# PrimeIntellect-ai/prime

Measured on AMD Instinct MI355X. Metric: tokens_per_sec, higher is better.
Workload: dtype bf16; 1 GPU; model=intellect_10b, global_batch=8, seq_len=2048, parallelism=diloco1_h100_int8ring

## Files before the change

### prime_amd/models/llama.py

```python
from __future__ import annotations

import math

import torch
import torch.nn as nn
import torch.nn.functional as F
from torch.utils.checkpoint import checkpoint

from .. import ops
from .configs import LlamaConfig, get_config


class PrimeLinear(nn.Linear):

    def forward(self, x):
        return ops.tuned_linear(x, self.weight)


class RMSNorm(nn.Module):
    def __init__(self, dim: int, eps: float):
        super().__init__()
        self.weight = nn.Parameter(torch.ones(dim))
        self.eps = eps

    def forward(self, x):
        return ops.rmsnorm(x, self.weight, self.eps)


class Attention(nn.Module):
    def __init__(self, cfg: LlamaConfig):
        super().__init__()
        self.cfg = cfg
        hd = cfg.head_dim
        self.wqkv = PrimeLinear(cfg.dim, (cfg.n_heads + 2 * cfg.n_kv_heads) * hd, bias=False)
        self.wo = PrimeLinear(cfg.n_heads * hd, cfg.dim, bias=False)

    sp_group = None

    def forward(self, x, cos, sin, cache=None, pos: int = 0, pos_dev=None):
        B, S, _ = x.shape
        cfg = self.cfg
        hd = cfg.head_dim
        qkv = self.wqkv(x)
        q, k, v = qkv.split(
            [cfg.n_heads * hd, cfg.n_kv_heads * hd, cfg.n_kv_heads * hd], dim=-1
        )
        q = q.view(B, S, cfg.n_heads, hd)
        k = k.view(B, S, cfg.n_kv_heads, hd)
        v = v.view(B, S, cfg.n_kv_heads, hd)
        p32 = pos_dev["pos32"] if pos_dev is not None else None
        q = ops.apply_rope(q, cos, sin, pos_offset=pos, pos_dev=p32)
        k = ops.apply_rope(k, cos, sin, pos_offset=pos, pos_dev=p32)
        if cache is not None:
            kc, vc = cache
            if pos_dev is not None:
                kc.index_copy_(1, pos_dev["pos64"], k)
                vc.index_copy_(1, pos_dev["pos64"], v)
                o = ops.attn_decode(q, kc, vc, length=1,
                                    len_dev=pos_dev["len32"])
                return self.wo(o.reshape(B, 1, cfg.n_heads * hd))
            kc[:, pos : pos + S] = k
            vc[:, pos : pos + S] = v
            if S == 1:
                o = ops.attn_decode(q, kc, vc, length=pos + 1)
                return self.wo(o.reshape(B, 1, cfg.n_heads * hd))
            o = ops.flash_attention(q, k, v, causal=True)
            return self.wo(o.reshape(B, S, cfg.n_heads * hd))
        if self.sp_group is not None:
            from ..parallel.seqpar import ulysses_attention

            o = ulysses_attention(q, k, v, causal=True, group=self.sp_group)
        else:
            o = ops.flash_attention(q, k, v, causal=True)
        return self.wo(o.reshape(B, S, cfg.n_heads * hd))


class MLP(nn.Module):
    def __init__(self, cfg: LlamaConfig):
        super().__init__()
        self.w_gateup = PrimeLinear(cfg.dim, 2 * cfg.intermediate, bias=False)
        self.w_down = PrimeLinear(cfg.intermediate, cfg.dim, bias=False)

    def forward(self, x):
        return self.w_down(ops.swiglu(self.w_gateup(x)))


class Block(nn.Module):

    def __init__(self, cfg: LlamaConfig):
        super().__init__()
        self.attn_norm = RMSNorm(cfg.dim, cfg.norm_eps)
        self.attn = Attention(cfg)
        self.mlp_norm = RMSNorm(cfg.dim, cfg.norm_eps)
        self.mlp = MLP(cfg)

    def forward(self, x, res, cos, sin, cache=None, pos: int = 0, pos_dev=None):
        y, s = ops.fused_add_rmsnorm(x, res, self.attn_norm.weight,
                                     self.attn_norm.eps)
        a = self.attn(y, cos, sin, cache=cache, pos=pos, pos_dev=pos_dev)
        y2, s2 = ops.fused_add_rmsnorm(a, s, self.mlp_norm.weight,
                                       self.mlp_norm.eps)
        return self.mlp(y2), s2


class Llama(nn.Module):
    def __init__(self, cfg: LlamaConfig, activation_checkpointing: bool = False):
        super().__init__()
# ... 58 lines not shown
```

### prime_amd/ops/__init__.py

```python
from .functional import (
    apply_rope,
    invalidate_wt_cache,
    set_linear_fp8,
    set_linear_tuned,
    tuned_linear,
    attn_decode,
    fused_add_rmsnorm,
    cross_entropy,
    dequant_int8,
    flash_attention,
    fused_adamw,
    grad_sqnorm,
    mfma_probe,
    nesterov_outer,
    pseudograd,
    quant_int8,
    rmsnorm,
    swiglu,
    QBLK,
)
from . import reference
from ._lib import have_lib
from .build import build, LIB_PATH

__all__ = [
    "apply_rope",
    "attn_decode",
    "fused_add_rmsnorm",
# ... 18 lines not shown
```

### prime_amd/ops/_lib.py

```python
from __future__ import annotations

import ctypes
from typing import Optional

import torch

from .build import LIB_PATH, build, needs_build

_LIB: Optional[ctypes.CDLL] = None
_TRIED = False

_SIGS = {
    "prime_rmsnorm_fwd": [ctypes.c_void_p] * 5 + [ctypes.c_int64] * 2 + [ctypes.c_double],
    "prime_rmsnorm_bwd": [ctypes.c_void_p] * 7 + [ctypes.c_int64] * 3 + [ctypes.c_double],
    "prime_add_rmsnorm_fwd": [ctypes.c_void_p] * 7 + [ctypes.c_int64] * 2 + [ctypes.c_double],
    "prime_add_rmsnorm_bwd": [ctypes.c_void_p] * 8 + [ctypes.c_int64] * 3 + [ctypes.c_double],
    "prime_rope": [ctypes.c_void_p] * 5 + [ctypes.c_int64] * 4 + [ctypes.c_int, ctypes.c_int64, ctypes.c_void_p],
    "prime_swiglu_fwd": [ctypes.c_void_p] * 3 + [ctypes.c_int64] * 2,
    "prime_swiglu_bwd": [ctypes.c_void_p] * 4 + [ctypes.c_int64] * 2,
    "prime_adamw": [ctypes.c_void_p] * 7 + [ctypes.c_int64] + [ctypes.c_double] * 5 + [ctypes.c_int64],
    "prime_grad_sqnorm": [ctypes.c_void_p] * 3 + [ctypes.c_int64] * 2,
    "prime_grad_sqnorm_partials": [],
    "prime_pseudograd": [ctypes.c_void_p] * 4 + [ctypes.c_int64],
    "prime_quant_int8": [ctypes.c_void_p] * 4 + [ctypes.c_int64],
    "prime_dequant_int8": [ctypes.c_void_p] * 4 + [ctypes.c_int64] * 2,
    "prime_nesterov_outer": [ctypes.c_void_p] * 6 + [ctypes.c_int64] + [ctypes.c_double] * 2,
    "prime_cross_entropy": [ctypes.c_void_p] * 5 + [ctypes.c_int64] * 2 + [ctypes.c_double] + [ctypes.c_int64] * 2,
    "prime_flash_fwd": [ctypes.c_void_p] * 6 + [ctypes.c_int64] * 5 + [ctypes.c_double] + [ctypes.c_int64] * 7,
    "prime_attn_delta": [ctypes.c_void_p] * 4 + [ctypes.c_int64] * 2,
    "prime_flash_bwd_dq": [ctypes.c_void_p] * 9 + [ctypes.c_int64] * 5 + [ctypes.c_double] + [ctypes.c_int64] * 10,
    "prime_flash_bwd_dkv": [ctypes.c_void_p] * 13 + [ctypes.c_int64] * 6 + [ctypes.c_double] + [ctypes.c_int64] * 10,
    "prime_mfma_probe": [ctypes.c_void_p] * 4,
    "prime_mfma_probe32": [ctypes.c_void_p] * 4,
    "prime_transpose_bshd": [ctypes.c_void_p] * 3 + [ctypes.c_int64] * 7,
    "prime_attn_decode": [ctypes.c_void_p] * 5 + [ctypes.c_int64] * 6 + [ctypes.c_double, ctypes.c_void_p],
    "prime_gemm_nt": [ctypes.c_void_p] * 4 + [ctypes.c_int64] * 4,
    "prime_gemm_nt8": [ctypes.c_void_p] * 4 + [ctypes.c_int64] * 4,
    "prime_quant_fp8": [ctypes.c_void_p] * 6 + [ctypes.c_int64] * 2,
    "prime_rowwise_quant_fp8": [ctypes.c_void_p] * 4 + [ctypes.c_int64] * 3,
    "prime_transpose_fp8": [ctypes.c_void_p] * 3 + [ctypes.c_int64] * 7 + [ctypes.c_void_p] * 3 + [ctypes.c_int64],
# ... 60 lines not shown
```

### prime_amd/ops/csrc/cross_entropy.hip

```cpp
#include "common.h"

__global__ void ce_fwd_bwd_kernel(const bf16* __restrict__ logits,
                                  const int32_t* __restrict__ targets,
                                  float* __restrict__ loss,
                                  bf16* __restrict__ dlogits, int64_t R, int V,
                                  float grad_scale, int ignore_index,
                                  int compute_grad) {
  __shared__ float red_m[256];
  __shared__ float red_s[256];
  const int tid = threadIdx.x;
  const int nthr = blockDim.x;
  const int vv = V / 8;
  for (int64_t r = blockIdx.x; r < R; r += gridDim.x) {
    const int tgt = targets[r];
    if (tgt == ignore_index) {
      if (tid == 0) loss[r] = 0.f;
      if (compute_grad) {
        bf16x8 z{};
#pragma unroll
        for (int j = 0; j < 8; ++j) z.v[j] = f2bf(0.f);
        bf16x8* dr = reinterpret_cast<bf16x8*>(dlogits + r * V);
        for (int i = tid; i < vv; i += nthr) dr[i] = z;
      }
      continue;
    }
    const bf16x8* zr = reinterpret_cast<const bf16x8*>(logits + r * V);
    float m = -INFINITY, s = 0.f;
    for (int i = tid; i < vv; i += nthr) {
      const bf16x8 z = zr[i];
#pragma unroll
      for (int j = 0; j < 8; ++j) {
        const float f = bf2f(z.v[j]);
        if (f > m) {
          s = s * __expf(m - f) + 1.f;
          m = f;
        } else {
          s += __expf(f - m);
        }
      }
    }
    red_m[tid] = m;
    red_s[tid] = s;
    __syncthreads();
    for (int stride = nthr / 2; stride > 0; stride >>= 1) {
      if (tid < stride) {
        const float m2 = red_m[tid + stride], s2 = red_s[tid + stride];
        const float mm = fmaxf(red_m[tid], m2);
        red_s[tid] = red_s[tid] * __expf(red_m[tid] - mm) + s2 * __expf(m2 - mm);
        red_m[tid] = mm;
      }
      __syncthreads();
    }
    const float M = red_m[0], S = red_s[0];
    __syncthreads();
    if (tid == 0) loss[r] = M + __logf(S) - bf2f(logits[r * V + tgt]);
    if (compute_grad) {
      const float invS = 1.f / S;
      bf16x8* dr = reinterpret_cast<bf16x8*>(dlogits + r * V);
      for (int i = tid; i < vv; i += nthr) {
        const bf16x8 z = zr[i];
        bf16x8 d;
#pragma unroll
        for (int j = 0; j < 8; ++j) {
          const int col = i * 8 + j;
          float p = __expf(bf2f(z.v[j]) - M) * invS;
          if (col == tgt) p -= 1.f;
          d.v[j] = f2bf(p * grad_scale);
        }
        dr[i] = d;
      }
    }
  }
// ... 16 lines not shown
```

### prime_amd/ops/csrc/rope.hip

```cpp
#include "common.h"

__global__ void rope_kernel(const bf16* __restrict__ x, bf16* __restrict__ y,
                            const float* __restrict__ cos_t,
                            const float* __restrict__ sin_t, int64_t nrows,
                            int H, int S, int D, float sign,
                            int64_t pos_offset,
                            const int* __restrict__ pos_dev) {
  if (pos_dev) pos_offset = *pos_dev;
  const int half = D / 2;
  const int hv = half / 4;
  const int64_t total = nrows * hv;
  for (int64_t idx = (int64_t)blockIdx.x * blockDim.x + threadIdx.x;
       idx < total; idx += (int64_t)gridDim.x * blockDim.x) {
    const int64_t row = idx / hv;
    const int i4 = (int)(idx - row * hv) * 4;
    const int64_t s = (row / H) % S + pos_offset;
    const bf16x4 x1 = *reinterpret_cast<const bf16x4*>(x + row * D + i4);
    const bf16x4 x2 = *reinterpret_cast<const bf16x4*>(x + row * D + half + i4);
    const f32x4v c = *reinterpret_cast<const f32x4v*>(cos_t + s * half + i4);
    const f32x4v sn = *reinterpret_cast<const f32x4v*>(sin_t + s * half + i4);
    bf16x4 y1, y2;
#pragma unroll
    for (int j = 0; j < 4; ++j) {
      const float a = bf2f(x1.v[j]), b = bf2f(x2.v[j]);
      const float sj = sign * sn.v[j];
      y1.v[j] = f2bf(a * c.v[j] - b * sj);
      y2.v[j] = f2bf(b * c.v[j] + a * sj);
    }
    *reinterpret_cast<bf16x4*>(y + row * D + i4) = y1;
    *reinterpret_cast<bf16x4*>(y + row * D + half + i4) = y2;
  }
}

PRIME_API int prime_rope(hipStream_t stream, const void* x, void* y,
                         const void* cos_t, const void* sin_t, int64_t nrows,
                         int64_t H, int64_t S, int64_t D, int backward,
                         int64_t pos_offset, const void* pos_dev) {
  if (D % 8 != 0) return hipErrorInvalidValue;
  int64_t total = nrows * (D / 8);
  int grid = prime_grid(total, 256);
  hipLaunchKernelGGL(rope_kernel, dim3(grid), dim3(256), 0, stream,
                     (const bf16*)x, (bf16*)y, (const float*)cos_t,
                     (const float*)sin_t, nrows, (int)H, (int)S, (int)D,
                     backward ? -1.f : 1.f, pos_offset, (const int*)pos_dev);
  return (int)hipGetLastError();
}
```

### prime_amd/ops/csrc/swiglu.hip

```cpp
#include "common.h"

__device__ __forceinline__ float sigmoidf_(float x) {
  return 1.f / (1.f + __expf(-x));
}

__global__ void swiglu_fwd_kernel(const bf16* __restrict__ gu,
                                  bf16* __restrict__ out, int64_t R, int I) {
  const int iv = I / 8;
  const int64_t total = R * iv;
  for (int64_t idx = (int64_t)blockIdx.x * blockDim.x + threadIdx.x;
       idx < total; idx += (int64_t)gridDim.x * blockDim.x) {
    const int64_t r = idx / iv;
    const int i = (int)(idx - r * iv) * 8;
    const bf16x8 g = *reinterpret_cast<const bf16x8*>(gu + r * 2 * I + i);
    const bf16x8 u = *reinterpret_cast<const bf16x8*>(gu + r * 2 * I + I + i);
    bf16x8 o;
#pragma unroll
    for (int j = 0; j < 8; ++j) {
      const float gf = bf2f(g.v[j]);
      o.v[j] = f2bf(gf * sigmoidf_(gf) * bf2f(u.v[j]));
    }
    *reinterpret_cast<bf16x8*>(out + r * I + i) = o;
  }
}

__global__ void swiglu_bwd_kernel(const bf16* __restrict__ dout,
                                  const bf16* __restrict__ gu,
                                  bf16* __restrict__ dgu, int64_t R, int I) {
  const int iv = I / 8;
  const int64_t total = R * iv;
  for (int64_t idx = (int64_t)blockIdx.x * blockDim.x + threadIdx.x;
       idx < total; idx += (int64_t)gridDim.x * blockDim.x) {
    const int64_t r = idx / iv;
    const int i = (int)(idx - r * iv) * 8;
    const bf16x8 g = *reinterpret_cast<const bf16x8*>(gu + r * 2 * I + i);
    const bf16x8 u = *reinterpret_cast<const bf16x8*>(gu + r * 2 * I + I + i);
    const bf16x8 d = *reinterpret_cast<const bf16x8*>(dout + r * I + i);
    bf16x8 dg, du;
#pragma unroll
    for (int j = 0; j < 8; ++j) {
      const float gf = bf2f(g.v[j]);
      const float sg = sigmoidf_(gf);
      const float silu = gf * sg;
      const float df = bf2f(d.v[j]);
      dg.v[j] = f2bf(df * bf2f(u.v[j]) * sg * (1.f + gf * (1.f - sg)));
      du.v[j] = f2bf(df * silu);
    }
    *reinterpret_cast<bf16x8*>(dgu + r * 2 * I + i) = dg;
    *reinterpret_cast<bf16x8*>(dgu + r * 2 * I + I + i) = du;
  }
}

PRIME_API int prime_swiglu_fwd(hipStream_t stream, const void* gu, void* out,
                               int64_t R, int64_t I) {
  if (I % 8 != 0) return hipErrorInvalidValue;
  int grid = prime_grid(R * (I / 8), 256);
  hipLaunchKernelGGL(swiglu_fwd_kernel, dim3(grid), dim3(256), 0, stream,
                     (const bf16*)gu, (bf16*)out, R, (int)I);
  return (int)hipGetLastError();
}

PRIME_API int prime_swiglu_bwd(hipStream_t stream, const void* dout,
                               const void* gu, void* dgu, int64_t R, int64_t I) {
  if (I % 8 != 0) return hipErrorInvalidValue;
  int grid = prime_grid(R * (I / 8), 256);
  hipLaunchKernelGGL(swiglu_bwd_kernel, dim3(grid), dim3(256), 0, stream,
                     (const bf16*)dout, (const bf16*)gu, (bf16*)dgu, R, (int)I);
  return (int)hipGetLastError();
}
```

### prime_amd/ops/functional.py

```python
from __future__ import annotations

import torch

from . import reference as ref
from ._lib import check, lib, ptr, stream_of

_DW_ROWS = 1024


def _is_hip(t: torch.Tensor) -> bool:
    return t.is_cuda


class _RMSNorm(torch.autograd.Function):
    @staticmethod
    def forward(ctx, x: torch.Tensor, w: torch.Tensor, eps: float):
        if not _is_hip(x):
            ctx.save_for_backward(x, w)
            ctx.eps = eps
            return ref.rmsnorm(x, w, eps)
        x = x.contiguous()
        shp = x.shape
        D = shp[-1]
        if D % 8 != 0:
# ... 30 lines not shown
        dx = torch.empty_like(x)
        G = max(1, min(R, _DW_ROWS))
        dw = torch.empty(G, D, device=x.device, dtype=torch.float32)
        check(
            lib().prime_rmsnorm_bwd(
                stream_of(x), ptr(dy), ptr(x), ptr(w), ptr(rstd), ptr(dx), ptr(dw), R, D, G, ctx.eps
            ),
            "rmsnorm_bwd",
        )
        return dx, dw.sum(0).to(w.dtype), None


def rmsnorm(x: torch.Tensor, w: torch.Tensor, eps: float = 1e-5) -> torch.Tensor:
    return _RMSNorm.apply(x, w, eps)


class _Rope(torch.autograd.Function):
    @staticmethod
    def forward(ctx, x, cos, sin, pos_offset: int, pos_dev=None):
        if not _is_hip(x):
            ctx.cpu = (cos, sin, pos_offset)
            return ref.apply_rope(x, cos, sin, pos_offset)
        ctx.cpu = None
        x = x.contiguous()
        B, S, H, D = x.shape
        y = torch.empty_like(x)
        check(
            lib().prime_rope(
                stream_of(x), ptr(x), ptr(y), ptr(cos), ptr(sin), B * S * H,
                H, S, D, 0, pos_offset, ptr(pos_dev),
            ),
            "rope_fwd",
        )
        ctx.save_for_backward(cos, sin)
        ctx.meta = (B, S, H, D, pos_offset)
        return y

    @staticmethod
    def backward(ctx, dy):
        if ctx.cpu is not None:
            cos, sin, off = ctx.cpu
            return ref.apply_rope(dy, cos, -sin, off), None, None, None, None
        cos, sin = ctx.saved_tensors
        B, S, H, D, off = ctx.meta
        dy = dy.contiguous()
        dx = torch.empty_like(dy)
        check(
            lib().prime_rope(
                stream_of(dy), ptr(dy), ptr(dx), ptr(cos), ptr(sin), B * S * H,
                H, S, D, 1, off, ptr(None),
            ),
            "rope_bwd",
        )
        return dx, None, None, None, None


def apply_rope(x, cos, sin, pos_offset: int = 0, pos_dev=None):
    return _Rope.apply(x, cos, sin, pos_offset, pos_dev)


class _SwiGLU(torch.autograd.Function):
    @staticmethod
    def forward(ctx, gu):
        if not _is_hip(gu):
            ctx.save_for_backward(gu)
            return ref.swiglu(gu)
        gu = gu.contiguous()
        I = gu.shape[-1] // 2
        if I % 8 != 0:
            raise NotImplementedError(
                f"swiglu kernel needs intermediate dim % 8 == 0 (got {I})"
            )
        R = gu.numel() // (2 * I)
        out = torch.empty(*gu.shape[:-1], I, device=gu.device, dtype=gu.dtype)
        check(lib().prime_swiglu_fwd(stream_of(gu), ptr(gu), ptr(out), R, I), "swiglu_fwd")
        ctx.save_for_backward(gu)
        return out

    @staticmethod
    def backward(ctx, dout):
        (gu,) = ctx.saved_tensors
        if not _is_hip(gu):
            g = gu.detach().float().requires_grad_(True)
            with torch.enable_grad():
                y = ref.swiglu(g)
            (gx,) = torch.autograd.grad(y, [g], dout.float())
            return gx.to(gu.dtype)
        dout = dout.contiguous()
        I = gu.shape[-1] // 2
        R = gu.numel() // (2 * I)
        dgu = torch.empty_like(gu)
        check(lib().prime_swiglu_bwd(stream_of(gu), ptr(dout), ptr(gu), ptr(dgu), R, I), "swiglu_bwd")
        return dgu


def swiglu(gu: torch.Tensor) -> torch.Tensor:
    return _SwiGLU.apply(gu)


def transpose_bshd(x: torch.Tensor) -> torch.Tensor:
    B, S, H, D = x.shape
    if not x.is_cuda or S % 64 != 0 or D % 64 != 0 or x.stride(3) != 1:
        return x.permute(0, 2, 3, 1).contiguous()
    out = torch.empty(B, H, D, S, device=x.device, dtype=x.dtype)
    check(
        lib().prime_transpose_bshd(
            stream_of(x), ptr(x), ptr(out), B, S, H, D,
            x.stride(0), x.stride(1), x.stride(2),
        ),
        "transpose_bshd",
    )
    return out


def _bshd_ok(t: torch.Tensor) -> bool:
    sb, ss, sh, sd = t.stride()
    return sd == 1 and sb % 8 == 0 and ss % 8 == 0 and sh % 8 == 0 \
        and t.storage_offset() % 8 == 0


def _check_flash_shape(S: int, D: int) -> None:
    if D not in (64, 128) or S % 64 != 0:
# ... 160 lines not shown
    M, C = x2.shape
    st = _FP8_ACT.get(site)
    import os

    fused_ok = os.environ.get("PRIME_AMD_FUSED_TQ", "0") == "1"
    if st is None or M % 64 or C % 128 or not fused_ok:
        xt = transpose_bshd(x2.view(1, M, C // 128, 128)).view(C, M)
        return _quant_act_fp8(xt, site, e5m2=e5m2)
    dt8 = torch.float8_e5m2 if e5m2 else torch.float8_e4m3fn
    xt8 = torch.empty(C, M, device=x2.device, dtype=dt8)
    st["next"].zero_()
    check(
        lib().prime_transpose_fp8(
            stream_of(x2), ptr(x2), ptr(xt8), 1, M, C // 128, 128,
            x2.stride(0) * M, x2.stride(0), 128,
            ptr(st["amax"]), ptr(st["next"]), ptr(st["sinv"]), 1 if e5m2 else 0,
        ),
        "transpose_fp8",
    )
    st["amax"], st["next"] = st["next"], st["amax"]
    return xt8, st["sinv"]


def _compute_dw(x2, w, dy2):
    N, K = w.shape
    M = x2.shape[0]
    if N % 128 == 0 and M % 64 == 0 and M >= 4096:
        if (_LINEAR_FP8_WGRAD and K % 128 == 0 and M % 16 == 0
                and x2.dtype == torch.bfloat16):
            xt8, xtinv = _transpose_quant_fp8(
                x2, ("xT", w.data_ptr(), *w.shape))
            dyt8, dytinv = _transpose_quant_fp8(
                dy2, ("dyT", w.data_ptr(), *w.shape), e5m2=True)
            g = torch._scaled_mm(xt8, dyt8.t(), scale_a=xtinv,
                                 scale_b=dytinv, out_dtype=x2.dtype)
            return transpose_bshd(g.view(1, K, N // 128, 128)).view(N, K)
        dyt = transpose_bshd(dy2.view(1, M, N // 128, 128)).view(N, M)
        return torch.mm(dyt, x2)
    return torch.mm(dy2.t(), x2)


def _linear_backward(x2, w, dy):
    N, K = w.shape
    M = x2.shape[0]
    dy2 = dy.reshape(-1, N).contiguous()
    wt = _wt_of(w) if _LINEAR_TUNED else None
    if (_LINEAR_FP8_DGRAD and wt is not None and M % 16 == 0
            and dy2.dtype == torch.bfloat16):
        dy8, dyinv = _quant_act_fp8(dy2, ("dy", w.data_ptr(), *w.shape),
                                    e5m2=True)
        wt8, wtinv = _w8_of(wt, skey=("wt", w.data_ptr(), *w.shape))
        dx = torch._scaled_mm(dy8, wt8.t(), scale_a=dyinv, scale_b=wtinv,
                              out_dtype=dy2.dtype)
    elif wt is not None:
        dx = torch.matmul(dy2, wt.t())
    else:
        dx = torch.matmul(dy2, w)
    return dx.view(*dy.shape[:-1], K), _compute_dw(x2, w, dy2)


class _TunedLinear(torch.autograd.Function):
    @staticmethod
# ... 98 lines not shown
class _Fp8Linear(torch.autograd.Function):
    @staticmethod
    def forward(ctx, x, w):
        x2 = x.reshape(-1, x.shape[-1]).contiguous()
        rw = _fp8_rowwise_on()
        if rw:
            x8, sxinv = _quant_rowwise_fp8(x2)
        else:
            x8, sxinv = _quant_act_fp8(x2, (w.data_ptr(), *w.shape))
        w8, swinv = _w8_of(w, rowwise=rw)
        y = torch._scaled_mm(x8, w8.t(), scale_a=sxinv, scale_b=swinv,
                             out_dtype=x.dtype)
        ctx.save_for_backward(x2, w)
        return y.view(*x.shape[:-1], w.shape[0])

    @staticmethod
    def backward(ctx, dy):
        x2, w = ctx.saved_tensors
        return _linear_backward(x2, w, dy)


def tuned_linear(x: torch.Tensor, w: torch.Tensor) -> torch.Tensor:
    if not _is_hip(x) or x.numel() // x.shape[-1] < 1024:
        return torch.nn.functional.linear(x, w)
    if _LINEAR_FP8 and x.shape[-1] % 16 == 0 and w.shape[0] % 16 == 0:
        return _Fp8Linear.apply(x, w)
    return _TunedLinear.apply(x, w)


def fused_adamw(p32, p16, grad, m, v, *, lr, beta1, beta2, eps, wd, step,
                gscale=None):
    check(
        lib().prime_adamw(
            stream_of(p32), ptr(p32), ptr(p16), ptr(grad), ptr(m), ptr(v),
            ptr(gscale), p32.numel(), lr, beta1, beta2, eps, wd, step,
        ),
        "adamw",
    )


def grad_sqnorm(grad: torch.Tensor, out: torch.Tensor) -> None:
    part = torch.zeros(lib().prime_grad_sqnorm_partials(), device=grad.device,
                       dtype=torch.float32)
    check(lib().prime_grad_sqnorm(stream_of(grad), ptr(grad), ptr(part),
                                  grad.numel(), part.numel()),
          "grad_sqnorm")
    out.add_(part.sum())


def pseudograd(outer32, master32, out_delta):
# ... 139 lines not shown
```

### prime_amd/parallel/flat.py

```python
from __future__ import annotations

from typing import Iterator

import torch
import torch.nn as nn

from .. import ops

ALIGN = 64


class FlatParamSpace:

    def __init__(self, module: nn.Module):
        self.module = module
        self.params: list[tuple[str, nn.Parameter]] = [
            (n, p) for n, p in module.named_parameters() if p.requires_grad
        ]
        if not self.params:
            raise ValueError("module has no trainable parameters")
        seen: dict[int, str] = {}
        uniq = []
        for n, p in self.params:
            if id(p) in seen:
# ... 3 lines not shown
        self.params = uniq

        dev = self.params[0][1].device
        dt = self.params[0][1].dtype
        self.device, self.dtype = dev, dt

        self.offsets: dict[str, tuple[int, int, torch.Size]] = {}
        off = 0
        for n, p in self.params:
            numel = p.numel()
            self.offsets[n] = (off, numel, p.shape)
            off += (numel + ALIGN - 1) // ALIGN * ALIGN
        self.numel_padded = off

        self.flat_w = torch.zeros(off, device=dev, dtype=dt)
        self.flat_grad = torch.zeros(off, device=dev, dtype=dt)
        for n, p in self.params:
            o, k, shp = self.offsets[n]
            self.flat_w[o : o + k].copy_(p.detach().flatten())
            p.data = self.flat_w[o : o + k].view(shp)
            p.grad = self.flat_grad[o : o + k].view(shp)
        self.master32 = self.flat_w.float()
        self._sq = None

    def zero_grad(self) -> None:
        self.flat_grad.zero_()

    def grad_views(self) -> Iterator[torch.Tensor]:
        for n, _ in self.params:
            o, k, shp = self.offsets[n]
            yield self.flat_grad[o : o + k].view(shp)

    def clip_grad_norm_(self, max_norm: float) -> torch.Tensor:
        norm = self.flat_grad.float().norm(2)
        scale = (max_norm / (norm + 1e-6)).clamp(max=1.0)
        self.flat_grad.mul_(scale.to(self.flat_grad.dtype))
        return norm

    def grad_clip_scale(self, max_norm: float) -> torch.Tensor:
        if self._sq is None:
            self._sq = torch.zeros(1, device=self.device, dtype=torch.float32)
        self._sq.zero_()
        ops.grad_sqnorm(self.flat_grad, self._sq)
        return (max_norm / (self._sq.sqrt() + 1e-6)).clamp(max=1.0)

    def state_dict(self) -> dict:
        return {"flat_w": self.flat_w, "master32": self.master32}

    def load_flat_(self, master32: torch.Tensor) -> None:
        self.master32.copy_(master32)
        self.flat_w.copy_(self.master32.to(self.dtype))
        ops.invalidate_wt_cache()


class FusedAdamW:

    def __init__(self, flat: FlatParamSpace, lr=3e-4, betas=(0.9, 0.95),
                 eps=1e-8, weight_decay=0.1):
        self.flat = flat
        self.lr, self.betas, self.eps, self.wd = lr, betas, eps, weight_decay
        self.m = torch.zeros_like(flat.master32)
        self.v = torch.zeros_like(flat.master32)
        self.step_count = 0

    def step(self, gscale=None) -> None:
# ... 30 lines not shown
```

### prime_amd/train.py

```python
from __future__ import annotations

import math
import os
import time
from pathlib import Path

import torch

from .ckpt.manager import CheckpointManager
from .data import DataConfig, build_dataloader
from .models import build_model
from .parallel.diloco import DilocoOptimizer
from .parallel.flat import FlatParamSpace, FusedAdamW
from .parallel.mesh import ElasticDeviceMesh, MeshConfig
from .utils.config import TrainConfig
from .utils.logging import JsonLogger
from .utils.metrics import MetricsWriter, model_flops_per_token, mfu


def lr_at(step: int, cfg) -> float:
    if step < cfg.warmup_steps:
        return cfg.lr * (step + 1) / max(1, cfg.warmup_steps)
    if not cfg.lr_decay_steps:
        return cfg.lr
# ... 67 lines not shown
        if self.fsdp:
            from .parallel.fsdp import ShardedParamSpace

            if not cfg.model.activation_checkpointing:
                self.model.activation_checkpointing = True
            self.flat = ShardedParamSpace(self.model, self.mesh)
            if self.mesh.outer_group is not None:
                import torch.distributed as dist

                dist.broadcast(self.flat.flat_w, src=self.mesh.worker_rank,
                               group=self.mesh.outer_group)
                self.flat.master32.copy_(self.flat.flat_w.float())
        else:
            self.flat = FlatParamSpace(self.model)
            if self.mesh.initialized:
                import torch.distributed as dist

                dist.broadcast(self.flat.flat_w, src=0)
                self.flat.master32.copy_(self.flat.flat_w.float())

        from . import ops as _ops

        _ops.set_linear_tuned(self.device.type == "cuda" and not self.fsdp)
        _ops.set_linear_fp8(cfg.model.fp8 and self.device.type == "cuda",
                            dgrad=cfg.model.fp8_dgrad,
                            wgrad=cfg.model.fp8_wgrad)

        self.inner = FusedAdamW(
            self.flat, lr=cfg.optim.lr, betas=tuple(cfg.optim.betas),
            eps=cfg.optim.eps, weight_decay=cfg.optim.weight_decay,
        )
        self.elastic = None
        self.shard_client = None
        if cfg.parallel.elastic and self.mesh.is_leader:
            from .parallel.elastic import ElasticWorker

            self.elastic = ElasticWorker(
                worker_name=cfg.run_name,
                host_store=os.environ.get("PRIME_GLOBAL_HOST", "0") == "1",
                heartbeat_interval=cfg.parallel.heartbeat_interval,
                heartbeat_timeout=cfg.parallel.heartbeat_timeout,
                ckpt_provider=lambda: self.diloco.live_state(),
            )
        elif cfg.parallel.elastic and self.fsdp:
            from .parallel.elastic import ElasticShardClient

# ... 60 lines not shown
            cfg.data.micro_batch_size * cfg.data.grad_accum * cfg.model.seq_len
            * max(1, self.mesh.world_size)
        )
        self.flops_per_token = model_flops_per_token(self.model_cfg, cfg.model.seq_len)

    def train_step(self) -> torch.Tensor:
        cfg = self.cfg
        self.inner.lr = lr_at(self.step_count, cfg.optim)
        self.flat.zero_grad()
        loss_acc = None
        for _ in range(cfg.data.grad_accum):
            x, y = self.data.next_batch(self.device)
            if self.seq_par:
                sl = cfg.model.seq_len
                r = self.mesh.worker_rank
                x = x[:, r * sl : (r + 1) * sl]
                y = y[:, r * sl : (r + 1) * sl]
            loss = self.model.loss(x, y) / cfg.data.grad_accum
            loss.backward()
            loss_acc = loss.detach() if loss_acc is None else loss_acc + loss.detach()
        if self.fsdp:
            self.flat.finalize_grads()
        else:
            self.mesh.local_allreduce_grad(self.flat.flat_grad)
        gscale = None
        if cfg.optim.grad_clip > 0:
            if self.device.type == "cuda" and not self.fsdp:
                gscale = self.flat.grad_clip_scale(cfg.optim.grad_clip)
            else:
                self.flat.clip_grad_norm_(cfg.optim.grad_clip)
        did_outer = self.diloco.step(gscale)
        self.step_count += 1
        if did_outer:
            self._maybe_checkpoint()
        return loss_acc

    def _maybe_checkpoint(self) -> None:
        if not self.ckpt or self.cfg.checkpoint.interval <= 0:
            return
        if self.diloco.outer_step_count % self.cfg.checkpoint.interval != 0:
            return
        if not (self.mesh.is_leader or self.fsdp):
            return
        self.save_checkpoint()

    def save_checkpoint(self) -> None:
# ... 175 lines not shown
```

Baseline: 16120 tokens/s.

## Fuse QKV rope and gate-up SwiGLU backward with transposed grads; write wgrads directly

Adds fused autograd paths for the QKV projection plus RoPE and the gate-up projection plus SwiGLU. Their backward kernels produce the packed gradient and its transpose in one pass, so the weight-gradient GEMM can consume it without a separate transpose. Linear weight gradients are written directly into slots of the flat gradient buffer, which skips a full zero of that buffer and an extra accumulate copy. The cost is more complex gradient bookkeeping (zero ranges, deferred finalize), with a risk of stale or wrong gradients if a slot is not cleared correctly.

```diff
diff --git a/prime_amd/models/llama.py b/prime_amd/models/llama.py
--- a/prime_amd/models/llama.py
+++ b/prime_amd/models/llama.py
@@ -41,6 +41,17 @@
         B, S, _ = x.shape
         cfg = self.cfg
         hd = cfg.head_dim
+        if cache is None and pos_dev is None:
+            q, k, v = ops.qkv_rope(x, self.wqkv.weight, cos, sin,
+                                   cfg.n_heads, cfg.n_kv_heads, hd,
+                                   pos_offset=pos)
+            if self.sp_group is not None:
+                from ..parallel.seqpar import ulysses_attention
+
+                o = ulysses_attention(q, k, v, causal=True, group=self.sp_group)
+            else:
+                o = ops.flash_attention(q, k, v, causal=True)
+            return self.wo(o.reshape(B, S, cfg.n_heads * hd))
         qkv = self.wqkv(x)
         q, k, v = qkv.split(
             [cfg.n_heads * hd, cfg.n_kv_heads * hd, cfg.n_kv_heads * hd], dim=-1
@@ -82,7 +93,7 @@
         self.w_down = PrimeLinear(cfg.intermediate, cfg.dim, bias=False)
 
     def forward(self, x):
-        return self.w_down(ops.swiglu(self.w_gateup(x)))
+        return self.w_down(ops.gateup_swiglu(x, self.w_gateup.weight))
 
 
 class Block(nn.Module):
diff --git a/prime_amd/ops/__init__.py b/prime_amd/ops/__init__.py
--- a/prime_amd/ops/__init__.py
+++ b/prime_amd/ops/__init__.py
@@ -3,7 +3,14 @@
     invalidate_wt_cache,
     set_linear_fp8,
     set_linear_tuned,
+    set_direct_wgrad,
+    direct_wgrad_enabled,
     tuned_linear,
+    gateup_swiglu,
+    qkv_rope,
+    qkv_grad_pack,
+    rope_packed_fwd,
+    swiglu_bwd_t,
     attn_decode,
     fused_add_rmsnorm,
     cross_entropy,
diff --git a/prime_amd/ops/_lib.py b/prime_amd/ops/_lib.py
--- a/prime_amd/ops/_lib.py
+++ b/prime_amd/ops/_lib.py
@@ -16,6 +16,9 @@
     "prime_add_rmsnorm_fwd": [ctypes.c_void_p] * 7 + [ctypes.c_int64] * 2 + [ctypes.c_double],
     "prime_add_rmsnorm_bwd": [ctypes.c_void_p] * 8 + [ctypes.c_int64] * 3 + [ctypes.c_double],
     "prime_rope": [ctypes.c_void_p] * 5 + [ctypes.c_int64] * 4 + [ctypes.c_int, ctypes.c_int64, ctypes.c_void_p],
+    "prime_rope_strided": [ctypes.c_void_p] * 5 + [ctypes.c_int64] * 7,
+    "prime_qkv_grad_pack": [ctypes.c_void_p] * 8 + [ctypes.c_int64] * 6,
+    "prime_swiglu_bwd_t": [ctypes.c_void_p] * 5 + [ctypes.c_int64] * 2,
     "prime_swiglu_fwd": [ctypes.c_void_p] * 3 + [ctypes.c_int64] * 2,
     "prime_swiglu_bwd": [ctypes.c_void_p] * 4 + [ctypes.c_int64] * 2,
     "prime_adamw": [ctypes.c_void_p] * 7 + [ctypes.c_int64] + [ctypes.c_double] * 5 + [ctypes.c_int64],
diff --git a/prime_amd/ops/csrc/cross_entropy.hip b/prime_amd/ops/csrc/cross_entropy.hip
--- a/prime_amd/ops/csrc/cross_entropy.hip
+++ b/prime_amd/ops/csrc/cross_entropy.hip
@@ -46,8 +46,10 @@
       if (tid < stride) {
         const float m2 = red_m[tid + stride], s2 = red_s[tid + stride];
         const float mm = fmaxf(red_m[tid], m2);
-        red_s[tid] = red_s[tid] * __expf(red_m[tid] - mm) + s2 * __expf(m2 - mm);
-        red_m[tid] = mm;
+        if (mm > -INFINITY) {
+          red_s[tid] = red_s[tid] * __expf(red_m[tid] - mm) + s2 * __expf(m2 - mm);
+          red_m[tid] = mm;
+        }
       }
       __syncthreads();
     }
diff --git a/prime_amd/ops/csrc/rope.hip b/prime_amd/ops/csrc/rope.hip
--- a/prime_amd/ops/csrc/rope.hip
+++ b/prime_amd/ops/csrc/rope.hip
@@ -1,4 +1,12 @@
 #include "common.h"
+
+__device__ __forceinline__ void rope_rot(bf16 x1, bf16 x2, float c, float sn,
+                                         float sign, bf16& y1, bf16& y2) {
+  const float a = bf2f(x1), b = bf2f(x2);
+  const float sj = sign * sn;
+  y1 = f2bf(a * c - b * sj);
+  y2 = f2bf(b * c + a * sj);
+}
 
 __global__ void rope_kernel(const bf16* __restrict__ x, bf16* __restrict__ y,
                             const float* __restrict__ cos_t,
@@ -21,12 +29,8 @@
     const f32x4v sn = *reinterpret_cast<const f32x4v*>(sin_t + s * half + i4);
     bf16x4 y1, y2;
 #pragma unroll
-    for (int j = 0; j < 4; ++j) {
-      const float a = bf2f(x1.v[j]), b = bf2f(x2.v[j]);
-      const float sj = sign * sn.v[j];
-      y1.v[j] = f2bf(a * c.v[j] - b * sj);
-      y2.v[j] = f2bf(b * c.v[j] + a * sj);
-    }
+    for (int j = 0; j < 4; ++j)
+      rope_rot(x1.v[j], x2.v[j], c.v[j], sn.v[j], sign, y1.v[j], y2.v[j]);
     *reinterpret_cast<bf16x4*>(y + row * D + i4) = y1;
     *reinterpret_cast<bf16x4*>(y + row * D + half + i4) = y2;
   }
@@ -45,3 +49,141 @@
                      backward ? -1.f : 1.f, pos_offset, (const int*)pos_dev);
   return (int)hipGetLastError();
 }
+
+__global__ void rope_strided_kernel(const bf16* __restrict__ x,
+                                    bf16* __restrict__ y,
+                                    const float* __restrict__ cos_t,
+                                    const float* __restrict__ sin_t,
+                                    int64_t nrows, int H, int S, int D,
+                                    int64_t in_stride, int64_t head_off,
+                                    float sign, int64_t pos_offset) {
+  const int half = D / 2;
+  const int hv = half / 4;
+  const int64_t total = nrows * hv;
+  for (int64_t idx = (int64_t)blockIdx.x * blockDim.x + threadIdx.x;
+       idx < total; idx += (int64_t)gridDim.x * blockDim.x) {
+    const int64_t row = idx / hv;
+    const int i4 = (int)(idx - row * hv) * 4;
+    const int64_t tok = row / H;
+    const int h = (int)(row - tok * H);
+    const int64_t s = tok % S + pos_offset;
+    const bf16* xr = x + tok * in_stride + head_off + (int64_t)h * D;
+    const bf16x4 x1 = *reinterpret_cast<const bf16x4*>(xr + i4);
+    const bf16x4 x2 = *reinterpret_cast<const bf16x4*>(xr + half + i4);
+    const f32x4v c = *reinterpret_cast<const f32x4v*>(cos_t + s * half + i4);
+    const f32x4v sn = *reinterpret_cast<const f32x4v*>(sin_t + s * half + i4);
+    bf16x4 y1, y2;
+#pragma unroll
+    for (int j = 0; j < 4; ++j)
+      rope_rot(x1.v[j], x2.v[j], c.v[j], sn.v[j], sign, y1.v[j], y2.v[j]);
+    *reinterpret_cast<bf16x4*>(y + row * D + i4) = y1;
+    *reinterpret_cast<bf16x4*>(y + row * D + half + i4) = y2;
+  }
+}
+
+PRIME_API int prime_rope_strided(hipStream_t stream, const void* x, void* y,
+                                 const void* cos_t, const void* sin_t,
+                                 int64_t nrows, int64_t H, int64_t S,
+                                 int64_t D, int64_t in_stride,
+                                 int64_t head_off, int64_t pos_offset) {
+  if (D % 8 != 0 || in_stride % 4 != 0 || head_off % 4 != 0 || H <= 0 ||
+      S <= 0)
+    return hipErrorInvalidValue;
+  int64_t total = nrows * (D / 8);
+  int grid = prime_grid(total, 256);
+  hipLaunchKernelGGL(rope_strided_kernel, dim3(grid), dim3(256), 0, stream,
+                     (const bf16*)x, (bf16*)y, (const float*)cos_t,
+                     (const float*)sin_t, nrows, (int)H, (int)S, (int)D,
+                     in_stride, head_off, 1.f, pos_offset);
+  return (int)hipGetLastError();
+}
+
+template <int D>
+__global__ __launch_bounds__(256) void qkv_grad_pack_kernel(
+    const bf16* __restrict__ dq, const bf16* __restrict__ dk,
+    const bf16* __restrict__ dv, bf16* __restrict__ dqkv,
+    bf16* __restrict__ dqkvt, const float* __restrict__ cos_t,
+    const float* __restrict__ sin_t, int64_t M, int H, int Hkv, int S,
+    float sign, int64_t pos_offset) {
+  constexpr int TPD = D + 8;
+  constexpr int HALF = D / 2;
+  constexpr int UPR = HALF / 8;
+  __shared__ bf16 tile[64][TPD];
+  const int NH = H + 2 * Hkv;
+  const int hh = blockIdx.x % NH;
+  const int64_t m0 = (int64_t)(blockIdx.x / NH) * 64;
+  const int64_t C = (int64_t)NH * D;
+  const bf16* src;
+  int sh, shn;
+  bool rot = true;
+  if (hh < H) { src = dq; sh = hh; shn = H; }
+  else if (hh < H + Hkv) { src = dk; sh = hh - H; shn = Hkv; }
+  else { src = dv; sh = hh - H - Hkv; shn = Hkv; rot = false; }
+  const int t = threadIdx.x;
+#pragma unroll
+  for (int i = 0; i < (64 * UPR) / 256; ++i) {
+    const int un = i * 256 + t;
+    const int r = un / UPR, i8 = (un % UPR) * 8;
+    const int64_t m = m0 + r;
+    const bf16* xr = src + (m * shn + sh) * D;
+    const bf16x8 x1 = *reinterpret_cast<const bf16x8*>(xr + i8);
+    const bf16x8 x2 = *reinterpret_cast<const bf16x8*>(xr + HALF + i8);
+    bf16x8 y1 = x1, y2 = x2;
+    if (rot) {
+      const int64_t s = m % S + pos_offset;
+      const float* cr = cos_t + s * HALF + i8;
+      const float* sr = sin_t + s * HALF + i8;
+      const f32x4v c0 = *reinterpret_cast<const f32x4v*>(cr);
+      const f32x4v c1 = *reinterpret_cast<const f32x4v*>(cr + 4);
+      const f32x4v s0 = *reinterpret_cast<const f32x4v*>(sr);
+      const f32x4v s1 = *reinterpret_cast<const f32x4v*>(sr + 4);
+#pragma unroll
+      for (int j = 0; j < 4; ++j) {
+        rope_rot(x1.v[j], x2.v[j], c0.v[j], s0.v[j], sign, y1.v[j], y2.v[j]);
+        rope_rot(x1.v[4 + j], x2.v[4 + j], c1.v[j], s1.v[j], sign,
+                 y1.v[4 + j], y2.v[4 + j]);
+      }
+    }
+    bf16* orow = dqkv + m * C + (int64_t)hh * D;
+    *reinterpret_cast<bf16x8*>(orow + i8) = y1;
+    *reinterpret_cast<bf16x8*>(orow + HALF + i8) = y2;
+    *reinterpret_cast<bf16x8*>(&tile[r][i8]) = y1;
+    *reinterpret_cast<bf16x8*>(&tile[r][HALF + i8]) = y2;
+  }
+  __syncthreads();
+#pragma unroll
+  for (int i = 0; i < (D * 8) / 256; ++i) {
+    const int un = i * 256 + t;
+    const int d = un >> 3, s8 = (un & 7) * 8;
+    bf16x8 v;
+#pragma unroll
+    for (int j = 0; j < 8; ++j) v.v[j] = tile[s8 + j][d];
+    *reinterpret_cast<bf16x8*>(dqkvt + ((int64_t)hh * D + d) * M + m0 + s8) = v;
+  }
+}
+
+PRIME_API int prime_qkv_grad_pack(hipStream_t stream, const void* dq,
+                                  const void* dk, const void* dv, void* dqkv,
+                                  void* dqkvt, const void* cos_t,
+                                  const void* sin_t, int64_t M, int64_t H,
+                                  int64_t Hkv, int64_t S, int64_t D,
+                                  int64_t pos_offset) {
+  if (M <= 0 || M % 64 != 0 || H <= 0 || Hkv <= 0 || S <= 0 ||
+      (D != 64 && D != 128))
+    return hipErrorInvalidValue;
+  const int64_t grid = (M / 64) * (H + 2 * Hkv);
+  if (grid > 0x7fffffff) return hipErrorInvalidValue;
+  if (D == 128)
+    hipLaunchKernelGGL((qkv_grad_pack_kernel<128>), dim3((int)grid), dim3(256),
+                       0, stream, (const bf16*)dq, (const bf16*)dk,
+                       (const bf16*)dv, (bf16*)dqkv, (bf16*)dqkvt,
+                       (const float*)cos_t, (const float*)sin_t, M, (int)H,
+                       (int)Hkv, (int)S, -1.f, pos_offset);
+  else
+    hipLaunchKernelGGL((qkv_grad_pack_kernel<64>), dim3((int)grid), dim3(256),
+                       0, stream, (const bf16*)dq, (const bf16*)dk,
+                       (const bf16*)dv, (bf16*)dqkv, (bf16*)dqkvt,
+                       (const float*)cos_t, (const float*)sin_t, M, (int)H,
+                       (int)Hkv, (int)S, -1.f, pos_offset);
+  return (int)hipGetLastError();
+}
diff --git a/prime_amd/ops/csrc/swiglu.hip b/prime_amd/ops/csrc/swiglu.hip
--- a/prime_amd/ops/csrc/swiglu.hip
+++ b/prime_amd/ops/csrc/swiglu.hip
@@ -24,6 +24,20 @@
   }
 }
 
+__device__ __forceinline__ void swiglu_bwd8(const bf16x8& g, const bf16x8& u,
+                                            const bf16x8& d, bf16x8& dg,
+                                            bf16x8& du) {
+#pragma unroll
+  for (int j = 0; j < 8; ++j) {
+    const float gf = bf2f(g.v[j]);
+    const float sg = sigmoidf_(gf);
+    const float silu = gf * sg;
+    const float df = bf2f(d.v[j]);
+    dg.v[j] = f2bf(df * bf2f(u.v[j]) * sg * (1.f + gf * (1.f - sg)));
+    du.v[j] = f2bf(df * silu);
+  }
+}
+
 __global__ void swiglu_bwd_kernel(const bf16* __restrict__ dout,
                                   const bf16* __restrict__ gu,
                                   bf16* __restrict__ dgu, int64_t R, int I) {
@@ -37,15 +51,7 @@
     const bf16x8 u = *reinterpret_cast<const bf16x8*>(gu + r * 2 * I + I + i);
     const bf16x8 d = *reinterpret_cast<const bf16x8*>(dout + r * I + i);
     bf16x8 dg, du;
-#pragma unroll
-    for (int j = 0; j < 8; ++j) {
-      const float gf = bf2f(g.v[j]);
-      const float sg = sigmoidf_(gf);
-      const float silu = gf * sg;
-      const float df = bf2f(d.v[j]);
-      dg.v[j] = f2bf(df * bf2f(u.v[j]) * sg * (1.f + gf * (1.f - sg)));
-      du.v[j] = f2bf(df * silu);
-    }
+    swiglu_bwd8(g, u, d, dg, du);
     *reinterpret_cast<bf16x8*>(dgu + r * 2 * I + i) = dg;
     *reinterpret_cast<bf16x8*>(dgu + r * 2 * I + I + i) = du;
   }
@@ -68,3 +74,62 @@
                      (const bf16*)dout, (const bf16*)gu, (bf16*)dgu, R, (int)I);
   return (int)hipGetLastError();
 }
+
+#define SWT_TP 72
+
+__global__ __launch_bounds__(256) void swiglu_bwd_t_kernel(
+    const bf16* __restrict__ dout, const bf16* __restrict__ gu,
+    bf16* __restrict__ dgu, bf16* __restrict__ dgut, int64_t R, int I) {
+  __shared__ bf16 tg[64][SWT_TP];
+  __shared__ bf16 tu[64][SWT_TP];
+  const int n_ct = I / 64;
+  const int ct = blockIdx.x % n_ct;
+  const int64_t rt = blockIdx.x / n_ct;
+  const int64_t r0 = rt * 64;
+  const int c0 = ct * 64;
+  const int t = threadIdx.x;
+#pragma unroll
+  for (int i = 0; i < 2; ++i) {
+    const int un = i * 256 + t;
+    const int r = un >> 3, c8 = (un & 7) * 8;
+    const int64_t row = r0 + r;
+    const bf16x8 g =
+        *reinterpret_cast<const bf16x8*>(gu + row * 2 * I + c0 + c8);
+    const bf16x8 u =
+        *reinterpret_cast<const bf16x8*>(gu + row * 2 * I + I + c0 + c8);
+    const bf16x8 d = *reinterpret_cast<const bf16x8*>(dout + row * I + c0 + c8);
+    bf16x8 dg, du;
+    swiglu_bwd8(g, u, d, dg, du);
+    *reinterpret_cast<bf16x8*>(dgu + row * 2 * I + c0 + c8) = dg;
+    *reinterpret_cast<bf16x8*>(dgu + row * 2 * I + I + c0 + c8) = du;
+    *reinterpret_cast<bf16x8*>(&tg[r][c8]) = dg;
+    *reinterpret_cast<bf16x8*>(&tu[r][c8]) = du;
+  }
+  __syncthreads();
+#pragma unroll
+  for (int i = 0; i < 2; ++i) {
+    const int un = i * 256 + t;
+    const int c = un >> 3, s8 = (un & 7) * 8;
+    bf16x8 vg, vu;
+#pragma unroll
+    for (int j = 0; j < 8; ++j) {
+      vg.v[j] = tg[s8 + j][c];
+      vu.v[j] = tu[s8 + j][c];
+    }
+    *reinterpret_cast<bf16x8*>(dgut + (int64_t)(c0 + c) * R + r0 + s8) = vg;
+    *reinterpret_cast<bf16x8*>(dgut + (int64_t)(I + c0 + c) * R + r0 + s8) = vu;
+  }
+}
+
+PRIME_API int prime_swiglu_bwd_t(hipStream_t stream, const void* dout,
+                                 const void* gu, void* dgu, void* dgut,
+                                 int64_t R, int64_t I) {
+  if (R <= 0 || I <= 0 || R % 64 != 0 || I % 64 != 0)
+    return hipErrorInvalidValue;
+  const int64_t grid = (R / 64) * (I / 64);
+  if (grid > 0x7fffffff || I > 0x3fffffff) return hipErrorInvalidValue;
+  hipLaunchKernelGGL(swiglu_bwd_t_kernel, dim3((int)grid), dim3(256), 0,
+                     stream, (const bf16*)dout, (const bf16*)gu, (bf16*)dgu,
+                     (bf16*)dgut, R, (int)I);
+  return (int)hipGetLastError();
+}
diff --git a/prime_amd/ops/functional.py b/prime_amd/ops/functional.py
--- a/prime_amd/ops/functional.py
+++ b/prime_amd/ops/functional.py
@@ -76,8 +76,13 @@
             ctx.cpu = (cos, sin, pos_offset)
             return ref.apply_rope(x, cos, sin, pos_offset)
         ctx.cpu = None
+        B, S, H, D = x.shape
+        if pos_dev is None and not x.is_contiguous() and _rope_view_ok(x):
+            y = rope_packed_fwd(x, cos, sin, pos_offset)
+            ctx.save_for_backward(cos, sin)
+            ctx.meta = (B, S, H, D, pos_offset)
+            return y
         x = x.contiguous()
-        B, S, H, D = x.shape
         y = torch.empty_like(x)
         check(
             lib().prime_rope(
@@ -111,6 +116,52 @@
 
 def apply_rope(x, cos, sin, pos_offset: int = 0, pos_dev=None):
     return _Rope.apply(x, cos, sin, pos_offset, pos_dev)
+
+
+def _rope_view_ok(x: torch.Tensor) -> bool:
+    B, S, H, D = x.shape
+    sb, ss, sh, sd = x.stride()
+    return (sd == 1 and sh == D and D % 8 == 0 and ss % 4 == 0
+            and (B == 1 or sb == S * ss) and x.storage_offset() % 4 == 0)
+
+
+def rope_packed_fwd(x, cos, sin, pos_offset: int = 0) -> torch.Tensor:
+    if not _rope_view_ok(x):
+        raise NotImplementedError(
+            f"rope_packed_fwd: unsupported view (shape {tuple(x.shape)}, "
+            f"strides {x.stride()})")
+    B, S, H, D = x.shape
+    y = torch.empty(B, S, H, D, device=x.device, dtype=x.dtype)
+    check(
+        lib().prime_rope_strided(
+            stream_of(x), ptr(x), ptr(y), ptr(cos), ptr(sin), B * S * H,
+            H, S, D, x.stride(1), 0, pos_offset,
+        ),
+        "rope_strided",
+    )
+    return y
+
+
+def qkv_grad_pack(dq, dk, dv, cos, sin, pos_offset: int = 0):
+    B, S, H, D = dq.shape
+    Hkv = dk.shape[2]
+    M = B * S
+    if D not in (64, 128) or M % 64 != 0:
+        raise NotImplementedError(
+            f"qkv_grad_pack needs head_dim in {{64, 128}} and tokens % 64 == 0 "
+            f"(got head_dim={D}, tokens={M})")
+    dq, dk, dv = dq.contiguous(), dk.contiguous(), dv.contiguous()
+    C = (H + 2 * Hkv) * D
+    dqkv = torch.empty(M, C, device=dq.device, dtype=dq.dtype)
+    dqkvt = torch.empty(C, M, device=dq.device, dtype=dq.dtype)
+    check(
+        lib().prime_qkv_grad_pack(
+            stream_of(dq), ptr(dq), ptr(dk), ptr(dv), ptr(dqkv), ptr(dqkvt),
+            ptr(cos), ptr(sin), M, H, Hkv, S, D, pos_offset,
+        ),
+        "qkv_grad_pack",
+    )
+    return dqkv, dqkvt
 
 
 class _SwiGLU(torch.autograd.Function):
@@ -152,6 +203,28 @@
     return _SwiGLU.apply(gu)
 
 
+def swiglu_bwd_t(dout: torch.Tensor, gu: torch.Tensor):
+    gu = gu.contiguous()
+    dout = dout.contiguous()
+    I = gu.shape[-1] // 2
+    R = gu.numel() // (2 * I)
+    dgu = torch.empty_like(gu)
+    if R % 64 == 0 and I % 64 == 0 and R > 0:
+        dgut = torch.empty(2 * I, R, device=gu.device, dtype=gu.dtype)
+        check(
+            lib().prime_swiglu_bwd_t(stream_of(gu), ptr(dout), ptr(gu),
+                                     ptr(dgu), ptr(dgut), R, I),
+            "swiglu_bwd_t",
+        )
+        return dgu, dgut
+    if I % 8 != 0:
+        raise NotImplementedError(
+            f"swiglu kernel needs intermediate dim % 8 == 0 (got {I})")
+    check(lib().prime_swiglu_bwd(stream_of(gu), ptr(dout), ptr(gu), ptr(dgu), R, I),
+          "swiglu_bwd")
+    return dgu, dgu.view(R, 2 * I).t().contiguous()
+
+
 def transpose_bshd(x: torch.Tensor) -> torch.Tensor:
     B, S, H, D = x.shape
     if not x.is_cuda or S % 64 != 0 or D % 64 != 0 or x.stride(3) != 1:
@@ -358,9 +431,62 @@
     return xt8, st["sinv"]
 
 
-def _compute_dw(x2, w, dy2):
+_DIRECT_WGRAD = False
+_WGRAD_SLOTS: dict = {}
+
+
+def set_direct_wgrad(on: bool) -> None:
+    global _DIRECT_WGRAD
+    _DIRECT_WGRAD = bool(on)
+
+
+def direct_wgrad_enabled() -> bool:
+    return _DIRECT_WGRAD
+
+
+def register_wgrad_slot(w: torch.Tensor, grad_view: torch.Tensor, owner):
+    slot = [grad_view, False, owner, False]
+    _WGRAD_SLOTS[(w.data_ptr(), *w.shape)] = slot
+    return slot
+
+
+def unregister_wgrad_slots(owner) -> None:
+    for k in [k for k, s in _WGRAD_SLOTS.items() if s[2] is owner]:
+        del _WGRAD_SLOTS[k]
+
+
+def _wgrad_take(w: torch.Tensor):
+    if not _WGRAD_SLOTS:
+        return None
+    slot = _WGRAD_SLOTS.get((w.data_ptr(), *w.shape))
+    if slot is None or not slot[1]:
+        return None
+    if slot[2]() is None:
+        del _WGRAD_SLOTS[(w.data_ptr(), *w.shape)]
+        return None
+    slot[1] = False
+    return slot[0]
+
+
+def _wgrad_release(w: torch.Tensor) -> None:
+    if not _WGRAD_SLOTS:
+        return
+    out = _wgrad_take(w)
+    if out is not None:
+        out.zero_()
+    elif torch.is_grad_enabled():
+        slot = _WGRAD_SLOTS.get((w.data_ptr(), *w.shape))
+        if slot is not None:
+            slot[3] = True
+
+
+def _compute_dw(x2, w, dy2, dyt=None):
     N, K = w.shape
     M = x2.shape[0]
+    out = _wgrad_take(w)
+    if out is not None and not (out.dtype == x2.dtype == dy2.dtype):
+        out.zero_()
+        out = None
     if N % 128 == 0 and M % 64 == 0 and M >= 4096:
         if (_LINEAR_FP8_WGRAD and K % 128 == 0 and M % 16 == 0
                 and x2.dtype == torch.bfloat16):
@@ -370,10 +496,17 @@
                 dy2, ("dyT", w.data_ptr(), *w.shape), e5m2=True)
             g = torch._scaled_mm(xt8, dyt8.t(), scale_a=xtinv,
                                  scale_b=dytinv, out_dtype=x2.dtype)
-            return transpose_bshd(g.view(1, K, N // 128, 128)).view(N, K)
-        dyt = transpose_bshd(dy2.view(1, M, N // 128, 128)).view(N, M)
-        return torch.mm(dyt, x2)
-    return torch.mm(dy2.t(), x2)
+            dw = transpose_bshd(g.view(1, K, N // 128, 128)).view(N, K)
+            if out is not None:
+                out.copy_(dw)
+                return None
+            return dw
+        if dyt is None:
+            dyt = transpose_bshd(dy2.view(1, M, N // 128, 128)).view(N, M)
+        dw = torch.mm(dyt, x2, out=out)
+    else:
+        dw = torch.mm(dyt if dyt is not None else dy2.t(), x2, out=out)
+    return None if out is not None else dw
 
 
 def _linear_backward(x2, w, dy):
@@ -518,10 +651,100 @@
 
 def tuned_linear(x: torch.Tensor, w: torch.Tensor) -> torch.Tensor:
     if not _is_hip(x) or x.numel() // x.shape[-1] < 1024:
+        _wgrad_release(w)
         return torch.nn.functional.linear(x, w)
     if _LINEAR_FP8 and x.shape[-1] % 16 == 0 and w.shape[0] % 16 == 0:
         return _Fp8Linear.apply(x, w)
     return _TunedLinear.apply(x, w)
+
+
+def _fused_layout_ok(x: torch.Tensor, w: torch.Tensor) -> bool:
+    if not (_LINEAR_TUNED and not _LINEAR_FP8 and _is_hip(x)):
+        return False
+    if x.dtype != torch.bfloat16 or w.dtype != torch.bfloat16 or w.dim() != 2:
+        return False
+    M = x.numel() // x.shape[-1]
+    return w.shape[0] % 128 == 0 and M % 64 == 0 and M >= 4096
+
+
+def _dx_of(dy2: torch.Tensor, w: torch.Tensor) -> torch.Tensor:
+    wt = _wt_of(w) if _LINEAR_TUNED else None
+    return torch.matmul(dy2, wt.t()) if wt is not None else torch.matmul(dy2, w)
+
+
+class _GateUpSwiGLU(torch.autograd.Function):
+
+    @staticmethod
+    def forward(ctx, x, w):
+        x2 = x.reshape(-1, x.shape[-1])
+        gu = torch.matmul(x2, w.t())
+        I = w.shape[0] // 2
+        out = torch.empty(x2.shape[0], I, device=x.device, dtype=x.dtype)
+        check(lib().prime_swiglu_fwd(stream_of(gu), ptr(gu), ptr(out),
+                                     x2.shape[0], I), "swiglu_fwd")
+        ctx.save_for_backward(x2, w, gu)
+        ctx.xshape = x.shape
+        return out.view(*x.shape[:-1], I)
+
+    @staticmethod
+    def backward(ctx, dout):
+        x2, w, gu = ctx.saved_tensors
+        dgu, dgut = swiglu_bwd_t(dout.reshape(-1, dout.shape[-1]), gu)
+        dx = _dx_of(dgu, w)
+        return dx.view(ctx.xshape), _compute_dw(x2, w, dgu, dyt=dgut)
+
+
+def gateup_swiglu(x: torch.Tensor, w: torch.Tensor) -> torch.Tensor:
+    if _fused_layout_ok(x, w):
+        return _GateUpSwiGLU.apply(x, w)
+    return swiglu(tuned_linear(x, w))
+
+
+class _QkvRope(torch.autograd.Function):
+
+    @staticmethod
+    def forward(ctx, x, w, cos, sin, H, Hkv, D, pos_offset):
+        B, S, K = x.shape
+        x2 = x.reshape(-1, K)
+        qkv = torch.matmul(x2, w.t()).view(B, S, -1)
+        q = rope_packed_fwd(qkv[..., : H * D].view(B, S, H, D), cos, sin,
+                            pos_offset)
+        k = rope_packed_fwd(
+            qkv[..., H * D : (H + Hkv) * D].view(B, S, Hkv, D), cos, sin,
+            pos_offset)
+        v = qkv[..., (H + Hkv) * D :].view(B, S, Hkv, D)
+        ctx.save_for_backward(x2, w, cos, sin)
+        ctx.meta = (B, S, K, H, Hkv, D, pos_offset)
+        return q, k, v
+
+    @staticmethod
+    def backward(ctx, dq, dk, dv):
+        x2, w, cos, sin = ctx.saved_tensors
+        B, S, K, H, Hkv, D, off = ctx.meta
+        if dq is None:
+            dq = x2.new_zeros(B, S, H, D)
+        if dk is None:
+            dk = x2.new_zeros(B, S, Hkv, D)
+        if dv is None:
+            dv = x2.new_zeros(B, S, Hkv, D)
+        dqkv, dqkvt = qkv_grad_pack(dq, dk, dv, cos, sin, off)
+        dx = _dx_of(dqkv, w)
+        return (dx.view(B, S, K), _compute_dw(x2, w, dqkv, dyt=dqkvt),
+                None, None, None, None, None, None)
+
+
+def qkv_rope(x, w, cos, sin, n_heads: int, n_kv_heads: int, head_dim: int,
+             pos_offset: int = 0):
+    H, Hkv, D = n_heads, n_kv_heads, head_dim
+    if (x.dim() == 3 and D in (64, 128) and w.shape[0] == (H + 2 * Hkv) * D
+            and _fused_layout_ok(x, w)):
+        return _QkvRope.apply(x, w, cos, sin, H, Hkv, D, pos_offset)
+    B, S = x.shape[0], x.shape[1]
+    qkv = tuned_linear(x, w)
+    q, k, v = qkv.split([H * D, Hkv * D, Hkv * D], dim=-1)
+    q = apply_rope(q.view(B, S, H, D), cos, sin, pos_offset=pos_offset)
+    k = apply_rope(k.view(B, S, Hkv, D), cos, sin, pos_offset=pos_offset)
+    return q, k, v.view(B, S, Hkv, D)
 
 
 def fused_adamw(p32, p16, grad, m, v, *, lr, beta1, beta2, eps, wd, step,
diff --git a/prime_amd/parallel/flat.py b/prime_amd/parallel/flat.py
--- a/prime_amd/parallel/flat.py
+++ b/prime_amd/parallel/flat.py
@@ -1,5 +1,6 @@
 from __future__ import annotations
 
+import weakref
 from typing import Iterator
 
 import torch
@@ -49,16 +50,82 @@
             p.grad = self.flat_grad[o : o + k].view(shp)
         self.master32 = self.flat_w.float()
         self._sq = None
+        self._register_direct_wgrad()
+
+    def _register_direct_wgrad(self) -> None:
+        from ..models.llama import PrimeLinear
+
+        uses: dict[int, int] = {}
+        for _, p in self.module.named_parameters(remove_duplicate=False):
+            uses[id(p)] = uses.get(id(p), 0) + 1
+        name_of = {id(p): n for n, p in self.params}
+        direct: list[tuple[int, int, str]] = []
+        for m in self.module.modules():
+            if not isinstance(m, PrimeLinear) or m.bias is not None:
+                continue
+            p = m.weight
+            n = name_of.get(id(p))
+            if n is None or p.dim() != 2 or uses[id(p)] != 1:
+                continue
+            o, k, _ = self.offsets[n]
+            direct.append((o, o + k, n))
+        direct.sort()
+        self.direct_ranges = [(a, b) for a, b, _ in direct]
+        self.zero_ranges: list[tuple[int, int]] = []
+        cur = 0
+        for a, b in self.direct_ranges:
+            if a > cur:
+                self.zero_ranges.append((cur, a))
+            cur = b
+        if cur < self.numel_padded:
+            self.zero_ranges.append((cur, self.numel_padded))
+        self._slots = []
+        self._direct_step = False
+        if self.device.type != "cuda":
+            return
+        self._owner = weakref.ref(self)
+        params = dict(self.params)
+        for a, b, n in direct:
+            p = params[n]
+            self._slots.append(ops.functional.register_wgrad_slot(
+                p, self.flat_grad[a:b].view(p.shape), self._owner))
+        weakref.finalize(self, ops.functional.unregister_wgrad_slots,
+                         self._owner)
 
     def zero_grad(self) -> None:
-        self.flat_grad.zero_()
+        if not (self._slots and ops.direct_wgrad_enabled()):
+            for s in self._slots:
+                s[1] = s[3] = False
+            self._direct_step = False
+            self.flat_grad.zero_()
+            return
+        for a, b in self.zero_ranges:
+            self.flat_grad[a:b].zero_()
+        for s in self._slots:
+            if s[3]:
+                s[0].zero_()
+                s[1] = s[3] = False
+            else:
+                s[1] = True
+        self._direct_step = True
+
+    def finalize_grads(self) -> None:
+        if not self._direct_step:
+            return
+        for s in self._slots:
+            if s[1]:
+                s[0].zero_()
+                s[1] = False
+        self._direct_step = False
 
     def grad_views(self) -> Iterator[torch.Tensor]:
+        self.finalize_grads()
         for n, _ in self.params:
             o, k, shp = self.offsets[n]
             yield self.flat_grad[o : o + k].view(shp)
 
     def clip_grad_norm_(self, max_norm: float) -> torch.Tensor:
+        self.finalize_grads()
         norm = self.flat_grad.float().norm(2)
         scale = (max_norm / (norm + 1e-6)).clamp(max=1.0)
         self.flat_grad.mul_(scale.to(self.flat_grad.dtype))
@@ -68,6 +135,7 @@
         if self._sq is None:
             self._sq = torch.zeros(1, device=self.device, dtype=torch.float32)
         self._sq.zero_()
+        self.finalize_grads()
         ops.grad_sqnorm(self.flat_grad, self._sq)
         return (max_norm / (self._sq.sqrt() + 1e-6)).clamp(max=1.0)
 
diff --git a/prime_amd/train.py b/prime_amd/train.py
--- a/prime_amd/train.py
+++ b/prime_amd/train.py
@@ -113,6 +113,7 @@
         from . import ops as _ops
 
         _ops.set_linear_tuned(self.device.type == "cuda" and not self.fsdp)
+        _ops.set_direct_wgrad(self.device.type == "cuda" and not self.fsdp)
         _ops.set_linear_fp8(cfg.model.fp8 and self.device.type == "cuda",
                             dgrad=cfg.model.fp8_dgrad,
                             wgrad=cfg.model.fp8_wgrad)
@@ -219,6 +220,7 @@
         if self.fsdp:
             self.flat.finalize_grads()
         else:
+            self.flat.finalize_grads()
             self.mesh.local_allreduce_grad(self.flat.flat_grad)
         gscale = None
         if cfg.optim.grad_clip > 0:
```

Result: faster. 16530 tokens/s, median of 6 (+2.5%).
